# alexrenz/AdaPM

Hardware: AMD Instinct MI355X
Metric: pull_push_ops_per_s (higher is better)
Workload: dtype fp32; 1 GPU; model=kge_complex_dim512, entities=10000000, relations=1000, dim=512, neg_samples=16, global_batch=16384, triples=90000000, parallelism=ps-async-dp1, fused_step=True, warmup_extra_steps=400

## Files before the change

### adapm_amd/__init__.py

```python
from __future__ import annotations

import threading
from typing import Optional

import numpy as np
import torch

try:
    from . import _C
except ImportError as e:
    raise ImportError(
        "adapm_amd native extension not built — run `python build.py` at the repo root"
    ) from e

from . import runtime as _rt
from .sampling import SamplingManager, make_distribution
from .sync import SyncManager

TECH_ALL = 0
TECH_REPLICATION_ONLY = 1
TECH_RELOCATION_ONLY = 2

_SETUP = {}

# ... 67 lines not shown
        )
        if cfg.get("locality_stats"):
            self._s.enable_locality_stats()
        if cfg.get("trace_keys") is not None:
            tk = cfg["trace_keys"]
            t = torch.tensor([-1], dtype=torch.int64) if tk == "all" else _to_key_tensor(tk)
            self._s.enable_key_trace(t)
        self._stats_out = cfg.get("stats_out")
        self.sampling: Optional[SamplingManager] = None
        self._sync = SyncManager(self._s, rt, max_per_sec=cfg["max_sync_per_sec"],
                                 time_intent_actions=cfg["time_intent_actions"])
        self._sync.start()
        self._local_barrier = threading.Barrier(max(1, cfg["num_threads"]))
        self._num_workers = max(1, cfg["num_threads"])
        self._shut = False


    def enable_sampling_support(self, scheme: str, with_replacement: bool, distribution: str,
                                min: int, max: int, counts=None, power: float = 0.75,
                                pool_size: int = 5_000, reuse_factor: int = 4):
        d = make_distribution(distribution, min, max, seed=self.rt.rank, counts=counts,
                              power=power, device=self.rt.device)
        self.sampling = SamplingManager(self._s, scheme, with_replacement, d, min, max,
                                        pool_size=pool_size, reuse_factor=reuse_factor)

    def barrier(self):
        if self.rt.world > 1:
            with self.rt.worker_group_lock:
                torch.distributed.barrier(group=self.rt.worker_group)

    def my_rank(self) -> int:
        return self.rt.rank

    def shutdown(self):
        if self._shut:
            return
        self._shut = True
        self._sync.request_stop()
        self._sync.join()
        self._final_report()
        _rt.shutdown_runtime()

    def _final_report(self):
        import os
        import sys

        st = self.stats()
# ... 248 lines not shown
```

### adapm_amd/csrc/core.cpp

```cpp
#include <torch/extension.h>
#include <ATen/Parallel.h>

#include <algorithm>
#include <atomic>
#include <condition_variable>
#include <cstring>
#include <limits>
#include <deque>
#include <map>
#include <queue>
#include <tuple>
#include <memory>
#include <mutex>
#include <random>
#include <thread>
#include <chrono>
#include <unordered_map>
#include <unordered_set>
#include <cstdio>
#include <vector>

#include "common.h"
#include "kernels.h"
#include "ops.h"

#ifdef ADAPM_WITH_HIP
#include <c10/hip/HIPStream.h>
#endif

extern "C" {
int adapm_host_arena_alloc(long long floats, int want_device_visible, void** host_ptr,
                           void** dev_ptr);
void adapm_host_arena_free(void* host_ptr, int was_device_visible);
}

namespace adapm {

namespace py = pybind11;

static void* current_stream(const torch::Device& dev) {
#ifdef ADAPM_WITH_HIP
  if (dev.is_cuda()) return (void*)c10::hip::getCurrentHIPStream(dev.index()).stream();
#endif
  return nullptr;
}


struct Slab {
  torch::Tensor buf;
  float* data = nullptr;
// ... 142 lines not shown
  std::vector<Key> keys;
};

struct ChannelState {
  std::mutex mu;
  std::deque<IntentReq> intent_queue;
  std::vector<IntentReq> future_intents;
  struct IntentExpiry {
    Clock end;
    int wid;
    std::shared_ptr<std::vector<Key>> keys;
    bool operator>(const IntentExpiry& o) const { return end > o.end; }
  };
  std::priority_queue<IntentExpiry, std::vector<IntentExpiry>, std::greater<>> intent_expiry;
  std::unordered_set<Key> replicas;
  std::unordered_map<Key, uint64_t> holders;
  std::deque<OutRec> out_queue;
  std::vector<RespRec> responses;
  std::unordered_map<Key, uint32_t> reloc_ctr;
  std::unordered_map<Key, int64_t> reloc_round;
  std::atomic<int64_t> rounds{0};
  int64_t idle_streak = 0;
  std::atomic<int64_t> idle2_events{0};
};


class Server {
 public:
  Server(int64_t num_keys, torch::Tensor lens, int rank, int world, int num_channels,
         int num_workers, std::string device, double capacity_factor, int techniques,
         bool location_caches, int64_t device_cap_floats = 0, int64_t host_spill_floats = 0,
         double sync_threshold = 0.0)
      : num_keys_(num_keys),
        rank_(rank),
        world_(world),
        nch_(num_channels),
        techniques_(techniques),
        use_loc_cache_(location_caches),
        sync_threshold_(sync_threshold),
        dev_(device) {
    TORCH_CHECK((nch_ & (nch_ - 1)) == 0, "num_channels must be a power of 2");
    {
      int hw = (int)std::thread::hardware_concurrency();
      int nt = std::max(1, std::min(hw / std::max(1, world_) - 2, 31));
      if (const char* e = getenv("ADAPM_PASS_THREADS")) nt = std::max(1, atoi(e));
      pass_pool_.want_threads = nt;
// ... 2119 lines not shown
  bool fused_plain_ok(void* st) {
    if (clocks_.size() != 1 || fused_multi_stream_) return false;
    if (!fused_marks_.defined()) {
      if (getenv("ADAPM_FUSED_ATOMIC")) {
        fused_multi_stream_ = true;
        return false;
      }
      fused_marks_ = torch::zeros({rowmark_words(num_keys_)},
                                  torch::TensorOptions().dtype(torch::kInt32).device(dev_));
      if (getenv("ADAPM_FUSED_STATS"))
        fused_shared_stat_ =
            torch::zeros({1}, torch::TensorOptions().dtype(torch::kInt64).device(dev_));
      fused_marks_stream_ = st;
      return true;
    }
    if (st == fused_marks_stream_) return true;
#ifdef ADAPM_WITH_HIP
    hipStreamSynchronize((hipStream_t)fused_marks_stream_);
#endif
    fused_multi_stream_ = true;
    return false;
  }

  torch::Tensor kge_step_fused(torch::Tensor keys_s, torch::Tensor keys_r, torch::Tensor keys_o,
                               torch::Tensor keys_neg, int64_t N, int64_t D, double lr,
                               double eps) {
    TORCH_CHECK(world_ == 1, "kge_step_fused requires a single rank (all keys local)");
    TORCH_CHECK(uniform_len_ == 2 * D, "kge_step_fused: store rows must be [emb|accum] = 2D");
    TORCH_CHECK(layout_identity_.load(), "kge_step_fused requires the identity layout");
    TORCH_CHECK(dev_.is_cuda(), "kge_step_fused is the GPU fast path");
    for (auto* t : {&keys_s, &keys_r, &keys_o, &keys_neg}) check_keys(*t);
    int64_t B = keys_s.numel();
    TORCH_CHECK(keys_r.numel() == B && keys_o.numel() == B && keys_neg.numel() == B * N);
    auto rng_check = [&](const torch::Tensor& t) { check_key_range(t); };
    rng_check(keys_s);
    rng_check(keys_r);
    rng_check(keys_o);
    rng_check(keys_neg);

    auto loss = torch::empty({B}, torch::TensorOptions().dtype(torch::kFloat32).device(dev_));
    auto ks = keys_s.to(dev_, true);
    auto kr = keys_r.to(dev_, true);
    auto ko = keys_o.to(dev_, true);
    auto kn = keys_neg.to(dev_, true);
    void* st = current_stream(dev_);
    {
      InflightGuard g(this);
      std::unique_lock<std::mutex> mg(fused_mu_);
      if (fused_plain_ok(st)) {
        RowMarkKeys mk{{ks.data_ptr<int64_t>(), kr.data_ptr<int64_t>(), ko.data_ptr<int64_t>(),
                        kn.data_ptr<int64_t>()},
                       {B, B, B, B * N},
                       4};
        auto* marks = reinterpret_cast<uint32_t*>(fused_marks_.data_ptr<int32_t>());
        rowmark_set_gpu(marks, mk, st);
        kge_complex_step_fused_gpu(
            slab_.data, mk.keys[0], mk.keys[1], mk.keys[2], mk.keys[3], loss.data_ptr<float>(),
            (int)B, (int)N, (int)D, Slab::padded(uniform_len_), world_, rank_, (float)lr,
            (float)eps, st, marks,
            fused_shared_stat_.defined()
                ? reinterpret_cast<unsigned long long*>(fused_shared_stat_.data_ptr<int64_t>())
                : nullptr);
        rowmark_clear_gpu(marks, mk, st);
        stat_fused_plain_ += 1;
      } else {
        mg.unlock();
        kge_complex_step_fused_gpu(slab_.data, ks.data_ptr<int64_t>(), kr.data_ptr<int64_t>(),
                                   ko.data_ptr<int64_t>(), kn.data_ptr<int64_t>(),
                                   loss.data_ptr<float>(), (int)B, (int)N, (int)D,
                                   Slab::padded(uniform_len_), world_, rank_, (float)lr,
                                   (float)eps, st);
        stat_fused_atomic_ += 1;
      }
    }
    int64_t total = 3 * B + B * N;
    stat_pull_keys_ += total;
    stat_pull_local_ += total;
    stat_push_keys_ += total;
    stat_push_local_ += total;
    stat_pulls_ += 1;
    stat_pushes_ += 1;
    return loss;
  }

  struct FusedResolve {
    std::vector<std::vector<int64_t>> offs;
    std::vector<int64_t> missed;
    int64_t b_hit = 0;
  };

  FusedResolve resolve_fused(const std::vector<std::pair<const int64_t*, int>>& arrs,
                             int64_t B) {
    FusedResolve out;
    const int na = (int)arrs.size();
    constexpr int64_t G = 1024;
    int64_t nchunks = (B + G - 1) / G;
    struct Part {
      std::vector<std::vector<int64_t>> offs;
      std::vector<int64_t> missed;
    };
    std::vector<Part> parts(nchunks);
    pass_pool_.run(nchunks, [&](int64_t c0, int64_t c1) {
      for (int64_t c = c0; c < c1; ++c) {
        Part& P = parts[c];
        P.offs.resize(na);
// ... 863 lines not shown
  if (prob.is_cuda()) {
    alias_draw_gpu(prob.data_ptr<float>(), alias.data_ptr<int32_t>(), prob.numel(),
                   (uint64_t)seed, N, out.data_ptr<int64_t>(), current_stream(prob.device()));
  } else {
    alias_draw_cpu(prob.data_ptr<float>(), alias.data_ptr<int32_t>(), prob.numel(),
                   (uint64_t)seed, N, out.data_ptr<int64_t>());
  }
  return out;
}

}

PYBIND11_MODULE(TORCH_EXTENSION_NAME, m) {
  using namespace adapm;
  m.def("hip_available", &hip_available);
  m.def("kge_complex_step", &kge_complex_step, py::call_guard<py::gil_scoped_release>());
  m.def("alias_draw", &alias_draw, py::call_guard<py::gil_scoped_release>());
  m.def("rescal_step", &rescal_step, py::call_guard<py::gil_scoped_release>());
  m.def("rescal_step_grouped", &rescal_step_grouped, py::call_guard<py::gil_scoped_release>());
  m.def("kge_complex_score", &kge_complex_score, py::call_guard<py::gil_scoped_release>());
  m.def("w2v_sgns_step", &w2v_sgns_step, py::call_guard<py::gil_scoped_release>());
  m.def("mf_update_step", &mf_update_step, py::call_guard<py::gil_scoped_release>());
  m.def("mf_loss", &mf_loss, py::call_guard<py::gil_scoped_release>());
  py::class_<Server>(m, "Server")
      .def(py::init<int64_t, torch::Tensor, int, int, int, int, std::string, double, int, bool,
                    int64_t, int64_t, double>(),
           py::arg("num_keys"), py::arg("value_lengths"), py::arg("rank"), py::arg("world"),
           py::arg("num_channels"), py::arg("num_workers"), py::arg("device"),
           py::arg("capacity_factor") = 2.0, py::arg("techniques") = 0,
           py::arg("location_caches") = true, py::arg("device_cap_floats") = 0,
           py::arg("host_spill_floats") = 0, py::arg("sync_threshold") = 0.0)
      .def("pull", &Server::pull, py::call_guard<py::gil_scoped_release>())
      .def("push", &Server::push, py::call_guard<py::gil_scoped_release>())
      .def("pull_if_local", &Server::pull_if_local, py::call_guard<py::gil_scoped_release>())
      .def("is_local", &Server::is_local)
      .def("intent", &Server::intent, py::call_guard<py::gil_scoped_release>())
      .def("advance_clock", &Server::advance_clock)
      .def("current_clock", &Server::current_clock)
      .def("worker_clocks", &Server::worker_clocks)
      .def("wait", &Server::wait, py::call_guard<py::gil_scoped_release>())
      .def("wait_all", &Server::wait_all, py::call_guard<py::gil_scoped_release>())
      .def("is_finished", &Server::is_finished)
      .def("round_counts", &Server::round_counts)
      .def("wait_rounds", &Server::wait_rounds, py::call_guard<py::gil_scoped_release>())
      .def("idle_counts", &Server::idle_counts)
      .def("wait_idle", &Server::wait_idle, py::call_guard<py::gil_scoped_release>())
      .def("set_intent_ahead", &Server::set_intent_ahead)
      .def("sync_collect", &Server::sync_collect, py::call_guard<py::gil_scoped_release>())
      .def("sync_process", &Server::sync_process, py::call_guard<py::gil_scoped_release>())
      .def("sync_respond", &Server::sync_respond, py::call_guard<py::gil_scoped_release>())
      .def("sync_apply", &Server::sync_apply, py::call_guard<py::gil_scoped_release>())
      .def("sync_finish", &Server::sync_finish, py::arg("ch"),
           py::arg("globally_idle") = false, py::call_guard<py::gil_scoped_release>())
      .def("fail", &Server::fail, py::call_guard<py::gil_scoped_release>())
      .def("failed_reason", &Server::failed_reason)
      .def("scan_local", &Server::scan_local, py::call_guard<py::gil_scoped_release>())
      .def("kge_step_fused", &Server::kge_step_fused, py::call_guard<py::gil_scoped_release>())
      .def("w2v_step_fused", &Server::w2v_step_fused, py::call_guard<py::gil_scoped_release>())
      .def("mf_step_fused", &Server::mf_step_fused, py::call_guard<py::gil_scoped_release>())
      .def("kge_step_fused_general", &Server::kge_step_fused_general,
           py::call_guard<py::gil_scoped_release>())
      .def("w2v_step_fused_general", &Server::w2v_step_fused_general,
           py::call_guard<py::gil_scoped_release>())
      .def("mf_step_fused_general", &Server::mf_step_fused_general,
           py::call_guard<py::gil_scoped_release>())
      .def("rebalance_spill", &Server::rebalance_spill, py::arg("max_moves") = 4096,
           py::call_guard<py::gil_scoped_release>())
      .def("key_tier", &Server::key_tier)
      .def("get_len", &Server::get_len)
      .def("uniform_len", &Server::uniform_len)
      .def("layout_identity", &Server::layout_identity)
      .def("num_keys", &Server::num_keys)
      .def("rank", &Server::rank)
      .def("world", &Server::world)
      .def("num_channels", &Server::num_channels)
      .def("owner_hint", &Server::owner_hint)
      .def("enable_locality_stats", &Server::enable_locality_stats)
      .def("enable_key_trace", &Server::enable_key_trace)
      .def("debug_key_state", &Server::debug_key_state)
      .def("debug_set_loc_cache", &Server::debug_set_loc_cache)
// ... 7 lines not shown
```

### adapm_amd/csrc/kernels.h

```cpp
#pragma once
#include <cstdint>

namespace adapm {

void kge_complex_step_gpu(const float* s, const float* r, const float* o, const float* neg,
                          float* ds, float* dr, float* do_, float* dneg, float* loss,
                          int B, int N, int D, float lr, float eps, void* stream);
void kge_complex_step_cpu(const float* s, const float* r, const float* o, const float* neg,
                          float* ds, float* dr, float* do_, float* dneg, float* loss,
                          int B, int N, int D, float lr, float eps);

struct RowMarkKeys {
  const int64_t* keys[4];
  int64_t n[4];
  int count;
};
inline int64_t rowmark_words(int64_t rows) { return (rows + 15) / 16; }
void rowmark_set_gpu(uint32_t* marks, const RowMarkKeys& ks, void* stream);
void rowmark_clear_gpu(uint32_t* marks, const RowMarkKeys& ks, void* stream);

void kge_complex_step_fused_gpu(float* slab, const int64_t* keys_s, const int64_t* keys_r,
                                const int64_t* keys_o, const int64_t* keys_neg, float* loss,
                                int B, int N, int D, int32_t plen, int world, int rank,
                                float lr, float eps, void* stream,
// ... 33 lines not shown
void w2v_sgns_step_gpu(const float* ctr, const float* ctx, const float* neg, float* dctr,
                       float* dctx, float* dneg, float* loss, int B, int N, int D, float lr,
                       float eps, void* stream);
void w2v_sgns_step_cpu(const float* ctr, const float* ctx, const float* neg, float* dctr,
                       float* dctx, float* dneg, float* loss, int B, int N, int D, float lr,
                       float eps);

void mf_update_step_gpu(const float* w, const float* h, const float* x, float* dw, float* dh,
                        float* loss, int B, int R, float lr, float lambda, float eps,
                        void* stream);
void mf_update_step_cpu(const float* w, const float* h, const float* x, float* dw, float* dh,
                        float* loss, int B, int R, float lr, float lambda, float eps);

void mf_loss_gpu(const float* w, const float* h, const float* x, float* out2, int B, int R,
                 float lambda, void* stream);
void mf_loss_cpu(const float* w, const float* h, const float* x, float* out2, int B, int R,
                 float lambda);

void alias_draw_gpu(const float* prob, const int32_t* alias, int64_t n, uint64_t seed,
                    int64_t N, int64_t* out, void* stream);
void alias_draw_cpu(const float* prob, const int32_t* alias, int64_t n, uint64_t seed,
                    int64_t N, int64_t* out);

}

namespace adapm {


void kge_complex_score_mfma_gpu(const float* s, const float* r, const float* cand,
                                float* scores, float* qbuf, int B, int E, int D, void* stream);

void mfma_grouped_gemm_gpu(const float* S, const float* W, const float* R, float* out,
                           const int* starts, int G, int D, int sstride, int wstride,
                           int64_t rstride, int out_rstride, int64_t ostride, int mode,
                           int total_tiles, void* stream);

void rescal_mid_gpu(const float* U, const float* o, const float* neg, float* do_, float* dneg,
                    float* Wm, float* loss, int B, int N, int D, float lr, float eps,
                    void* stream);

void adagrad_rows_gpu(const float* grad, const float* rows, float* out, int64_t n_rows,
                      int dvals, int gstride, int rstride, float lr, float eps, void* stream);

}
```

### adapm_amd/csrc/kernels_cpu.cpp

```cpp
#include <cmath>
#include <vector>

#include "kernels.h"

namespace adapm {

static inline float sigmoidf_(float x) { return 1.f / (1.f + std::exp(-x)); }
static inline float softplusf_(float x) { return x > 20.f ? x : std::log1p(std::exp(x)); }

void kge_complex_step_cpu(const float* s, const float* r, const float* o, const float* neg,
                          float* ds, float* dr, float* do_, float* dneg, float* loss, int B,
                          int N, int D, float lr, float eps) {
  const int dc = D >> 1;
  const int row = D << 1;
  std::vector<float> a_sre(dc), a_sim(dc), a_rre(dc), a_rim(dc), u_re(dc), u_im(dc);
  for (int b = 0; b < B; ++b) {
    const float* sb = s + (int64_t)b * row;
    const float* rb = r + (int64_t)b * row;
    for (int k = 0; k < dc; ++k) {
      u_re[k] = sb[k] * rb[k] - sb[dc + k] * rb[dc + k];
      u_im[k] = sb[dc + k] * rb[k] + sb[k] * rb[dc + k];
      a_sre[k] = a_sim[k] = a_rre[k] = a_rim[k] = 0.f;
    }
    float lsum = 0.f;
    for (int j = 0; j <= N; ++j) {
      const float* ob = (j == 0) ? o + (int64_t)b * row : neg + ((int64_t)b * N + (j - 1)) * row;
// ... 239 lines not shown
    reg += lambda * nrm;
  }
  out2[0] += (float)se;
  out2[1] += (float)reg;
}

static inline uint64_t pcg_hash64_c(uint64_t x) {
  x ^= x >> 33; x *= 0xff51afd7ed558ccdULL;
  x ^= x >> 33; x *= 0xc4ceb9fe1a85ec53ULL;
  x ^= x >> 33;
  return x;
}

void alias_draw_cpu(const float* prob, const int32_t* alias, int64_t n, uint64_t seed,
                    int64_t N, int64_t* out) {
  for (int64_t i = 0; i < N; ++i) {
    uint64_t h = pcg_hash64_c(seed ^ (uint64_t)i * 0x9e3779b97f4a7c15ULL);
    int64_t slot = (int64_t)(h % (uint64_t)n);
    float u = (float)((h >> 40) & 0xffffff) * (1.0f / 16777216.0f);
    out[i] = (u < prob[slot]) ? slot : (int64_t)alias[slot];
  }
}

}

namespace adapm {

void rescal_step_cpu(const float* s, const float* r, const float* o, const float* neg,
                     float* ds, float* drl, float* do_, float* dneg, float* loss, int B, int N,
                     int D, float lr, float eps) {
  const int erow = 2 * D;
  const int64_t rrow = 2LL * D * D;
  std::vector<float> u(D), w(D), t(D);
  for (int b = 0; b < B; ++b) {
    const float* sb = s + (int64_t)b * erow;
    const float* rb = r + (int64_t)b * rrow;
    for (int j = 0; j < D; ++j) {
      double a = 0;
      for (int i = 0; i < D; ++i) a += rb[(int64_t)i * D + j] * sb[i];
      u[j] = (float)a;
    }
    std::fill(w.begin(), w.end(), 0.f);
    float lsum = 0.f;
    for (int j = 0; j <= N; ++j) {
      const float* ob = (j == 0) ? o + (int64_t)b * erow : neg + ((int64_t)b * N + j - 1) * erow;
      float* dob = (j == 0) ? do_ + (int64_t)b * erow : dneg + ((int64_t)b * N + j - 1) * erow;
// ... 36 lines not shown
```

### adapm_amd/csrc/kernels_hip.hip

```cpp
#include <hip/hip_runtime.h>
#include <algorithm>

#include "kernels.h"

namespace adapm {

#define KT 256

__device__ inline float block_reduce_sum(float v, float* lds) {
  for (int off = 32; off > 0; off >>= 1) v += __shfl_xor(v, off, 64);
  int wave = threadIdx.x >> 6;
  int lane = threadIdx.x & 63;
  if (lane == 0) lds[wave] = v;
  __syncthreads();
  float r = (threadIdx.x < KT / 64) ? lds[threadIdx.x] : 0.f;
  if (threadIdx.x < 64) {
    for (int off = 2; off > 0; off >>= 1) r += __shfl_xor(r, off, 64);
  }
  if (threadIdx.x == 0) lds[0] = r;
  __syncthreads();
  float out = lds[0];
  __syncthreads();
  return out;
}

__device__ inline float sigmoidf(float x) { return 1.f / (1.f + __expf(-x)); }
// ... 306 lines not shown
#undef LAUNCH
}
void mf_update_step_gpu(const float* w, const float* h, const float* x, float* dw, float* dh,
                        float* loss, int B, int R, float lr, float lambda, float eps,
                        void* stream) {
  hipLaunchKernelGGL(k_mf_step, dim3(grid_for(B)), dim3(KT), 0, (hipStream_t)stream, w, h, x, dw,
                     dh, loss, B, R, lr, lambda, eps);
}

}

namespace adapm {
void alias_draw_gpu(const float* prob, const int32_t* alias, int64_t n, uint64_t seed,
                    int64_t N, int64_t* out, void* stream) {
  if (N == 0) return;
  int blocks = (int)std::min<int64_t>((N + 255) / 256, 4096);
  hipLaunchKernelGGL(k_alias_draw, dim3(blocks), dim3(256), 0, (hipStream_t)stream, prob, alias,
                     n, seed, N, out);
}
}

namespace adapm {

__global__ void k_rescal_step(const float* __restrict__ s, const float* __restrict__ r,
                              const float* __restrict__ o, const float* __restrict__ neg,
                              float* __restrict__ ds, float* __restrict__ drl,
                              float* __restrict__ do_, float* __restrict__ dneg,
                              float* __restrict__ loss, int B, int N, int D, float lr,
                              float eps) {
  extern __shared__ __attribute__((aligned(16))) float smem[];
  float* Rm = smem;
  float* u = Rm + D * D;
  float* w = u + D;
  float* es = w + D;
  float* red = es + D;
  const int erow = 2 * D;
  const int64_t rrow = 2LL * D * D;

  for (int b = blockIdx.x; b < B; b += gridDim.x) {
    const float* sb = s + (int64_t)b * erow;
    const float* rb = r + (int64_t)b * rrow;
    for (int i = threadIdx.x; i < D * D; i += KT) Rm[i] = rb[i];
    for (int i = threadIdx.x; i < D; i += KT) {
      es[i] = sb[i];
      w[i] = 0.f;
    }
// ... 391 lines not shown
```

### adapm_amd/models/kge.py

```python
from __future__ import annotations

import dataclasses
import os
import time
from collections import defaultdict
from typing import Optional

import numpy as np
import torch

_PHASE_TIMING = os.environ.get("ADAPM_PHASE_TIMING", "0") == "1"

import adapm_amd
from adapm_amd import _C


@dataclasses.dataclass
class ComplExConfig:
    num_entities: int = 1_000_000
    num_relations: int = 1_000
    dim: int = 512
    neg_samples: int = 16
    batch_size: int = 4096
    lr: float = 0.1
    eps: float = 1e-6
    lookahead: int = 4
    init_scale: float = 0.1
    seed: int = 42

    @property
    def num_keys(self) -> int:
        return self.num_entities + self.num_relations

    @property
# ... 99 lines not shown
        pt = w.push(all_keys, all_d, async_=True)
        if pt != -1:
            self._pending.append(pt)
        if not async_push:
            w.wait(pt)
        while len(self._pending) > 64:
            w.wait(self._pending.pop(0))
        t0 = self._ph("push", t0)
        if sync_loss:
            out = float(loss.mean().item())
            self._ph("loss_sync", t0)
            return out
        return loss

    def train_batch_fused(self, triples: np.ndarray, sync_loss: bool = False,
                          force_general: bool = False):
        cfg = self.cfg
        w = self.worker
        raw = self.server.raw
        if self.dev.type != "cuda" and not force_general:
            return self.train_batch(triples, sync_loss=sync_loss)
        B = len(triples)
        s_keys, r_keys, o_keys = self.keys_of(triples)
        neg_keys = np.ascontiguousarray(self._draw_negatives(B), dtype=np.int64)

        if self.world == 1 and not force_general and raw.layout_identity():
            loss = raw.kge_step_fused(
                torch.from_numpy(s_keys), torch.from_numpy(r_keys), torch.from_numpy(o_keys),
                torch.from_numpy(neg_keys), cfg.neg_samples, cfg.dim, cfg.lr, cfg.eps)
            return float(loss.mean().item()) if sync_loss else loss

        negs2 = neg_keys.reshape(B, cfg.neg_samples)
        if self._deferred is not None:
            dtr, dng = self._deferred
            self._deferred = None
            n_def = len(dtr)
            triples = np.concatenate([dtr, triples])
            negs2 = np.concatenate([dng, negs2])
            s_keys, r_keys, o_keys = self.keys_of(triples)
            neg_keys = negs2.reshape(-1)
        else:
            n_def = 0

        loss, missed = raw.kge_step_fused_general(
            torch.from_numpy(s_keys), torch.from_numpy(r_keys), torch.from_numpy(o_keys),
            torch.from_numpy(np.ascontiguousarray(neg_keys)), cfg.neg_samples, cfg.dim,
            cfg.lr, cfg.eps)
        if missed.numel() == 0:
            return float(loss.mean().item()) if sync_loss else loss
# ... 390 lines not shown
```

### adapm_amd/sampling.py

```python
from __future__ import annotations

import threading
from dataclasses import dataclass, field
from typing import Dict, Optional

import numpy as np
import torch


class Distribution:
    def draw(self, n: int) -> np.ndarray:
        raise NotImplementedError


class Uniform(Distribution):
    def __init__(self, lo: int, hi: int, seed: int):
        self.lo, self.hi = lo, hi
        self.rng = np.random.default_rng(seed)

    def draw(self, n):
        return self.rng.integers(self.lo, self.hi, size=n, dtype=np.int64)


class LogUniform(Distribution):

    def __init__(self, lo: int, hi: int, seed: int):
        self.lo, self.hi = lo, hi
        self.rng = np.random.default_rng(seed)

    def draw(self, n):
        u = self.rng.random(n)
        k = np.exp(u * np.log(self.hi - self.lo + 1)) + self.lo - 1
        return np.minimum(k.astype(np.int64), self.hi - 1)


class Unigram(Distribution):

    def __init__(self, counts: np.ndarray, key_of: Optional[np.ndarray], power: float, seed: int,
                 device=None):
        p = counts.astype(np.float64) ** power
        p = p / p.sum()
        self.prob, self.alias = self._build_alias(p)
        self.key_of = key_of
        self.seed = np.random.default_rng(seed).integers(1, 2 ** 62)
# ... 20 lines not shown
        return (_t.from_numpy(prob.clip(0, 1).astype(np.float32)),
                _t.from_numpy(alias))

    def draw(self, n):
        from . import _C

        self._calls += 1
        out = _C.alias_draw(self.prob, self.alias, int(self.seed + self._calls), n)
        keys = out.cpu().numpy() if out.is_cuda else out.numpy()
        return keys if self.key_of is None else self.key_of[keys]


@dataclass
class _Sample:
    keys: Optional[np.ndarray]
    remaining: int
    used: set = field(default_factory=set)
    cursor: int = 0


class SamplingManager:

    def __init__(self, server, scheme: str, with_replacement: bool, dist_: Distribution,
                 lo: int, hi: int, pool_size: int = 5_000, reuse_factor: int = 4):
        self.POOL_SIZE = pool_size
        self.POOL_REUSE = reuse_factor
        self.server = server
        self.scheme = scheme
        self.with_replacement = with_replacement
        self.dist = dist_
        self.lo, self.hi = lo, hi
        self.lock = threading.Lock()
        self.samples: Dict[int, _Sample] = {}
        self.next_id = 1
        self.pool: np.ndarray = np.empty(0, dtype=np.int64)
        self.pool_uses = 0


    def prepare(self, worker, K: int, start: int, end: int) -> int:
        with self.lock:
            sid = self.next_id
            self.next_id += 1
        if self.scheme in ("naive", "preloc", "pool"):
            if self.scheme == "pool":
                keys = self._from_pool(K)
            else:
                keys = self._draw(K)
            self.samples[sid] = _Sample(keys=keys, remaining=K)
            if self.scheme == "preloc" and self.server.world() > 1:
                worker.intent(torch.from_numpy(keys), start, end)
        else:
            self.samples[sid] = _Sample(keys=None, remaining=K)
        return sid

    def pull(self, worker, sid: int, n: int):
        s = self.samples[sid]
        if s.remaining < n:
            raise ValueError(f"sample {sid}: requested {n} > remaining {s.remaining}")
        if self.scheme == "local":
            keys = self._local_draw(n, s)
        else:
            keys = s.keys[s.cursor:s.cursor + n]
            s.cursor += n
        s.remaining -= n
        return keys

    def finish(self, sid: int):
        self.samples.pop(sid, None)


    def _draw(self, n) -> np.ndarray:
        if self.with_replacement:
            return self.dist.draw(n)
        out = []
        seen = set()
        while len(out) < n:
            cand = self.dist.draw(max(2 * (n - len(out)), 16))
            for c in cand:
                c = int(c)
                if c not in seen:
                    seen.add(c)
                    out.append(c)
                    if len(out) == n:
                        break
        return np.array(out, dtype=np.int64)

    def _from_pool(self, n) -> np.ndarray:
        with self.lock:
            if len(self.pool) < n or self.pool_uses >= self.POOL_REUSE * self.POOL_SIZE:
                self.pool = self.dist.draw(max(self.POOL_SIZE, n))
                self.pool_uses = 0
# ... 43 lines not shown
```

Measured before the change: 941.9 million key-ops/s.

## Generate uniform negative samples on GPU with a bit-exact PCG64 stream

Adds a native UniformStream that reproduces numpy's PCG64 bounded-integer draw on the GPU using jump-ahead tables, a per-chunk generate kernel and a compaction kernel. The fused KGE step can then draw B*N negatives on the device instead of generating them in numpy and copying them over. Positive keys are also packed into one pinned buffer with a single range check and a single host-to-device copy, replacing four separate copies and checks. The price is substantial new RNG and state-sync code, plus stream-ownership synchronisation whenever RNG state moves between host and device.

Result: faster. 1.083 billion key-ops/s (median of 6 runs) (+15.0%).

```diff
diff --git a/adapm_amd/__init__.py b/adapm_amd/__init__.py
--- a/adapm_amd/__init__.py
+++ b/adapm_amd/__init__.py
@@ -113,7 +113,8 @@
         d = make_distribution(distribution, min, max, seed=self.rt.rank, counts=counts,
                               power=power, device=self.rt.device)
         self.sampling = SamplingManager(self._s, scheme, with_replacement, d, min, max,
-                                        pool_size=pool_size, reuse_factor=reuse_factor)
+                                        pool_size=pool_size, reuse_factor=reuse_factor,
+                                        device=self.rt.device)
 
     def barrier(self):
         if self.rt.world > 1:
diff --git a/adapm_amd/csrc/core.cpp b/adapm_amd/csrc/core.cpp
--- a/adapm_amd/csrc/core.cpp
+++ b/adapm_amd/csrc/core.cpp
@@ -23,9 +23,12 @@
 #include "common.h"
 #include "kernels.h"
 #include "ops.h"
+#include "ustream.h"
 
 #ifdef ADAPM_WITH_HIP
 #include <c10/hip/HIPStream.h>
+#include <ATen/core/CachingHostAllocator.h>
+#include <ATen/hip/impl/HIPStreamMasqueradingAsCUDA.h>
 #endif
 
 extern "C" {
@@ -214,6 +217,100 @@
   std::atomic<int64_t> rounds{0};
   int64_t idle_streak = 0;
   std::atomic<int64_t> idle2_events{0};
+};
+
+
+class UniformStream {
+ public:
+  UniformStream(int64_t lo, int64_t hi, const std::string& device)
+      : lo_(lo), hi_(hi), dev_(device) {
+    TORCH_CHECK(supported(lo, hi), "UniformStream: [", lo, ", ", hi,
+                ") is not a range of numpy's 32-bit bounded draw");
+    excl_ = (uint32_t)((uint64_t)hi - (uint64_t)lo);
+    thr_ = (uint32_t)((0x100000000ull - excl_) % excl_);
+    state_ = torch::zeros({USTREAM_STATE_WORDS},
+                          torch::TensorOptions().dtype(torch::kInt64).device(dev_));
+  }
+
+  static bool supported(int64_t lo, int64_t hi) {
+    if (hi <= lo || lo == std::numeric_limits<int64_t>::min()) return false;
+    uint64_t span = (uint64_t)hi - (uint64_t)lo;
+    return span >= 2 && span <= 0xFFFFFFFFull;
+  }
+
+  void import_state(uint64_t state_hi, uint64_t state_lo, uint64_t inc_hi, uint64_t inc_lo,
+                    uint64_t has_uint32, uint64_t uinteger) {
+    auto h = torch::empty({USTREAM_STATE_WORDS}, torch::kInt64);
+    uint64_t* p = reinterpret_cast<uint64_t*>(h.data_ptr<int64_t>());
+    p[0] = state_hi, p[1] = state_lo, p[2] = inc_hi, p[3] = inc_lo;
+    p[4] = has_uint32 ? 1 : 0, p[5] = uinteger & 0xFFFFFFFFull;
+    ustream_build_table(p);
+    std::lock_guard<std::mutex> g(mu_);
+    adopt(current_stream(dev_));
+    state_.copy_(h);
+  }
+
+  std::vector<uint64_t> export_state() {
+    torch::Tensor h;
+    {
+      std::lock_guard<std::mutex> g(mu_);
+      adopt(current_stream(dev_));
+      h = state_.slice(0, 0, USTREAM_GEN_WORDS).cpu();
+    }
+    const uint64_t* p = reinterpret_cast<const uint64_t*>(h.data_ptr<int64_t>());
+    return std::vector<uint64_t>(p, p + USTREAM_GEN_WORDS);
+  }
+
+  torch::Tensor draw(int64_t n, int64_t slack = -1) {
+    TORCH_CHECK(n >= 0, "UniformStream.draw: n must be >= 0");
+    auto opt = torch::TensorOptions().dtype(torch::kInt64).device(dev_);
+    auto out = torch::empty({n}, opt);
+    if (n == 0) return out;
+    if (slack < 0) {
+      double p = (double)thr_ / 4294967296.0;
+      double w0 = (double)n / (1.0 - p);
+      slack = (int64_t)std::ceil(w0 - (double)n + 8.0 * std::sqrt(w0 * p) / (1.0 - p)) + 16;
+    }
+    const int64_t words = n + slack;
+    std::lock_guard<std::mutex> g(mu_);
+    void* st = current_stream(dev_);
+    adopt(st);
+    auto tmp = torch::empty({ustream_tmp_words(words)}, opt);
+    uint64_t* sp = reinterpret_cast<uint64_t*>(state_.data_ptr<int64_t>());
+    if (dev_.is_cuda()) {
+#ifdef ADAPM_WITH_HIP
+      uniform_draw_gpu(sp, lo_, excl_, thr_, n, words, out.data_ptr<int64_t>(),
+                       tmp.data_ptr<int64_t>(), st);
+#else
+      TORCH_CHECK(false, "UniformStream: built without HIP");
+#endif
+    } else {
+      uniform_draw_cpu(sp, lo_, excl_, thr_, n, words, out.data_ptr<int64_t>(),
+                       tmp.data_ptr<int64_t>());
+    }
+    return out;
+  }
+
+  int64_t lo() const { return lo_; }
+  int64_t hi() const { return hi_; }
+  const torch::Device& device() const { return dev_; }
+
+ private:
+  void adopt(void* st) {
+#ifdef ADAPM_WITH_HIP
+    if (dev_.is_cuda() && have_owner_ && st != owner_) hipStreamSynchronize((hipStream_t)owner_);
+#endif
+    owner_ = st;
+    have_owner_ = true;
+  }
+
+  int64_t lo_, hi_;
+  uint32_t excl_ = 0, thr_ = 0;
+  torch::Device dev_;
+  torch::Tensor state_;
+  std::mutex mu_;
+  void* owner_ = nullptr;
+  bool have_owner_ = false;
 };
 
 
@@ -2379,36 +2476,89 @@
     return false;
   }
 
-  torch::Tensor kge_step_fused(torch::Tensor keys_s, torch::Tensor keys_r, torch::Tensor keys_o,
-                               torch::Tensor keys_neg, int64_t N, int64_t D, double lr,
-                               double eps) {
+  struct StagedKeys {
+    torch::Tensor dev;
+    std::vector<const int64_t*> ptr;
+  };
+  StagedKeys stage_keys(std::initializer_list<const torch::Tensor*> parts) {
+    int64_t total = 0;
+    for (auto* t : parts) {
+      check_keys(*t);
+      total += t->numel();
+    }
+    auto blob = torch::empty(
+        {total}, torch::TensorOptions().dtype(torch::kInt64).pinned_memory(true));
+    int64_t* dst = blob.data_ptr<int64_t>();
+    const uint64_t lim = (uint64_t)num_keys_;
+    uint64_t bad = 0;
+    for (auto* t : parts) {
+      const int64_t* kp = t->data_ptr<int64_t>();
+      const int64_t n = t->numel();
+      for (int64_t i = 0; i < n; ++i) {
+        int64_t k = kp[i];
+        dst[i] = k;
+        bad |= ((uint64_t)k >= lim);
+      }
+      dst += n;
+    }
+    if (bad)
+      for (auto* t : parts) check_key_range(*t);
+    StagedKeys sk;
+    sk.dev = torch::empty({total}, torch::TensorOptions().dtype(torch::kInt64).device(dev_));
+#ifdef ADAPM_WITH_HIP
+    auto stream = c10::hip::getCurrentHIPStreamMasqueradingAsCUDA(dev_.index());
+    TORCH_CHECK(copy_keys_gpu(sk.dev.data_ptr<int64_t>(), blob.data_ptr<int64_t>(), total,
+                              (void*)stream.stream()),
+                "kge_step_fused: the pinned key staging buffer is not visible to the device");
+    at::getHostAllocator(at::kCUDA)->record_event(
+        blob.data_ptr(), blob.storage().data_ptr().get_context(), stream.unwrap());
+#else
+    TORCH_CHECK(false, "kge_step_fused: built without HIP");
+#endif
+    const int64_t* dp = sk.dev.data_ptr<int64_t>();
+    for (auto* t : parts) {
+      sk.ptr.push_back(dp);
+      dp += t->numel();
+    }
+    return sk;
+  }
+
+  std::tuple<torch::Tensor, torch::Tensor> kge_step_fused_impl(
+      const torch::Tensor& keys_s, const torch::Tensor& keys_r, const torch::Tensor& keys_o,
+      const torch::Tensor* keys_neg, UniformStream* us, int64_t N, int64_t D, double lr,
+      double eps) {
     TORCH_CHECK(world_ == 1, "kge_step_fused requires a single rank (all keys local)");
     TORCH_CHECK(uniform_len_ == 2 * D, "kge_step_fused: store rows must be [emb|accum] = 2D");
     TORCH_CHECK(layout_identity_.load(), "kge_step_fused requires the identity layout");
     TORCH_CHECK(dev_.is_cuda(), "kge_step_fused is the GPU fast path");
-    for (auto* t : {&keys_s, &keys_r, &keys_o, &keys_neg}) check_keys(*t);
     int64_t B = keys_s.numel();
-    TORCH_CHECK(keys_r.numel() == B && keys_o.numel() == B && keys_neg.numel() == B * N);
-    auto rng_check = [&](const torch::Tensor& t) { check_key_range(t); };
-    rng_check(keys_s);
-    rng_check(keys_r);
-    rng_check(keys_o);
-    rng_check(keys_neg);
+    TORCH_CHECK(keys_r.numel() == B && keys_o.numel() == B);
+    StagedKeys sk;
+    torch::Tensor drawn;
+    const int64_t* kn;
+    if (us) {
+      TORCH_CHECK(us->lo() >= 0 && us->hi() <= num_keys_, "kge_step_fused_sampled: stream range [",
+                  us->lo(), ", ", us->hi(), ") exceeds the store's ", num_keys_, " keys");
+      TORCH_CHECK(us->device() == dev_,
+                  "kge_step_fused_sampled: stream is not on the store's device");
+      TORCH_CHECK(N >= 0 && B * N > 0, "kge_step_fused_sampled: nothing to draw");
+      sk = stage_keys({&keys_s, &keys_r, &keys_o});
+      drawn = us->draw(B * N);
+      kn = drawn.data_ptr<int64_t>();
+    } else {
+      TORCH_CHECK(keys_neg->numel() == B * N);
+      sk = stage_keys({&keys_s, &keys_r, &keys_o, keys_neg});
+      kn = sk.ptr[3];
+    }
+    const int64_t *ks = sk.ptr[0], *kr = sk.ptr[1], *ko = sk.ptr[2];
 
     auto loss = torch::empty({B}, torch::TensorOptions().dtype(torch::kFloat32).device(dev_));
-    auto ks = keys_s.to(dev_, true);
-    auto kr = keys_r.to(dev_, true);
-    auto ko = keys_o.to(dev_, true);
-    auto kn = keys_neg.to(dev_, true);
     void* st = current_stream(dev_);
     {
       InflightGuard g(this);
       std::unique_lock<std::mutex> mg(fused_mu_);
       if (fused_plain_ok(st)) {
-        RowMarkKeys mk{{ks.data_ptr<int64_t>(), kr.data_ptr<int64_t>(), ko.data_ptr<int64_t>(),
-                        kn.data_ptr<int64_t>()},
-                       {B, B, B, B * N},
-                       4};
+        RowMarkKeys mk{{ks, kr, ko, kn}, {B, B, B, B * N}, 4};
         auto* marks = reinterpret_cast<uint32_t*>(fused_marks_.data_ptr<int32_t>());
         rowmark_set_gpu(marks, mk, st);
         kge_complex_step_fused_gpu(
@@ -2422,11 +2572,9 @@
         stat_fused_plain_ += 1;
       } else {
         mg.unlock();
-        kge_complex_step_fused_gpu(slab_.data, ks.data_ptr<int64_t>(), kr.data_ptr<int64_t>(),
-                                   ko.data_ptr<int64_t>(), kn.data_ptr<int64_t>(),
-                                   loss.data_ptr<float>(), (int)B, (int)N, (int)D,
-                                   Slab::padded(uniform_len_), world_, rank_, (float)lr,
-                                   (float)eps, st);
+        kge_complex_step_fused_gpu(slab_.data, ks, kr, ko, kn, loss.data_ptr<float>(), (int)B,
+                                   (int)N, (int)D, Slab::padded(uniform_len_), world_, rank_,
+                                   (float)lr, (float)eps, st);
         stat_fused_atomic_ += 1;
       }
     }
@@ -2437,7 +2585,20 @@
     stat_push_local_ += total;
     stat_pulls_ += 1;
     stat_pushes_ += 1;
-    return loss;
+    return {loss, drawn};
+  }
+
+  torch::Tensor kge_step_fused(torch::Tensor keys_s, torch::Tensor keys_r, torch::Tensor keys_o,
+                               torch::Tensor keys_neg, int64_t N, int64_t D, double lr,
+                               double eps) {
+    return std::get<0>(
+        kge_step_fused_impl(keys_s, keys_r, keys_o, &keys_neg, nullptr, N, D, lr, eps));
+  }
+
+  std::tuple<torch::Tensor, torch::Tensor> kge_step_fused_sampled(
+      torch::Tensor keys_s, torch::Tensor keys_r, torch::Tensor keys_o, UniformStream& us,
+      int64_t N, int64_t D, double lr, double eps) {
+    return kge_step_fused_impl(keys_s, keys_r, keys_o, nullptr, &us, N, D, lr, eps);
   }
 
   struct FusedResolve {
@@ -3347,6 +3508,16 @@
   m.def("w2v_sgns_step", &w2v_sgns_step, py::call_guard<py::gil_scoped_release>());
   m.def("mf_update_step", &mf_update_step, py::call_guard<py::gil_scoped_release>());
   m.def("mf_loss", &mf_loss, py::call_guard<py::gil_scoped_release>());
+  py::class_<UniformStream>(m, "UniformStream")
+      .def(py::init<int64_t, int64_t, std::string>(), py::arg("lo"), py::arg("hi"),
+           py::arg("device"))
+      .def_static("supported", &UniformStream::supported)
+      .def("import_state", &UniformStream::import_state, py::call_guard<py::gil_scoped_release>())
+      .def("export_state", &UniformStream::export_state, py::call_guard<py::gil_scoped_release>())
+      .def("draw", &UniformStream::draw, py::arg("n"), py::arg("slack") = -1,
+           py::call_guard<py::gil_scoped_release>())
+      .def("lo", &UniformStream::lo)
+      .def("hi", &UniformStream::hi);
   py::class_<Server>(m, "Server")
       .def(py::init<int64_t, torch::Tensor, int, int, int, int, std::string, double, int, bool,
                     int64_t, int64_t, double>(),
@@ -3381,6 +3552,8 @@
       .def("failed_reason", &Server::failed_reason)
       .def("scan_local", &Server::scan_local, py::call_guard<py::gil_scoped_release>())
       .def("kge_step_fused", &Server::kge_step_fused, py::call_guard<py::gil_scoped_release>())
+      .def("kge_step_fused_sampled", &Server::kge_step_fused_sampled,
+           py::call_guard<py::gil_scoped_release>())
       .def("w2v_step_fused", &Server::w2v_step_fused, py::call_guard<py::gil_scoped_release>())
       .def("mf_step_fused", &Server::mf_step_fused, py::call_guard<py::gil_scoped_release>())
       .def("kge_step_fused_general", &Server::kge_step_fused_general,
diff --git a/adapm_amd/csrc/kernels.h b/adapm_amd/csrc/kernels.h
--- a/adapm_amd/csrc/kernels.h
+++ b/adapm_amd/csrc/kernels.h
@@ -79,6 +79,13 @@
 void alias_draw_cpu(const float* prob, const int32_t* alias, int64_t n, uint64_t seed,
                     int64_t N, int64_t* out);
 
+void uniform_draw_gpu(uint64_t* state, int64_t lo, uint32_t excl, uint32_t thr, int64_t n,
+                      int64_t words, int64_t* out, int64_t* tmp, void* stream);
+void uniform_draw_cpu(uint64_t* state, int64_t lo, uint32_t excl, uint32_t thr, int64_t n,
+                      int64_t words, int64_t* out, int64_t* tmp);
+
+bool copy_keys_gpu(int64_t* dst, const int64_t* src_host, int64_t n, void* stream);
+
 }
 
 namespace adapm {
diff --git a/adapm_amd/csrc/kernels_cpu.cpp b/adapm_amd/csrc/kernels_cpu.cpp
--- a/adapm_amd/csrc/kernels_cpu.cpp
+++ b/adapm_amd/csrc/kernels_cpu.cpp
@@ -1,7 +1,9 @@
+#include <algorithm>
 #include <cmath>
 #include <vector>
 
 #include "kernels.h"
+#include "ustream.h"
 
 namespace adapm {
 
@@ -287,6 +289,31 @@
   }
 }
 
+void uniform_draw_cpu(uint64_t* state, int64_t lo, uint32_t excl, uint32_t thr, int64_t n,
+                      int64_t words, int64_t* out, int64_t* tmp) {
+  const UStreamRange r{lo, excl, thr};
+  const int64_t chunks = ustream_chunks(words), nb = ustream_blocks(words);
+  int64_t* counts = tmp + USTREAM_TMP_COUNTS;
+  int64_t* keys = counts + nb;
+  for (int64_t b = 0; b < nb; ++b) counts[b] = 0;
+  for (int64_t c = 0; c < chunks; ++c)
+    counts[c / USTREAM_BLOCK] +=
+        ustream_gen_chunk(state, r, words, c, keys + c * USTREAM_CHUNK, 1);
+  int64_t total = 0, consumed = 0;
+  for (int64_t b = 0; b < nb; ++b) {
+    int64_t idx = total;
+    total += counts[b];
+    if (idx >= n) continue;
+    const int64_t w1 = std::min((b + 1) * (int64_t)USTREAM_BLOCK * USTREAM_CHUNK, words);
+    for (int64_t w = b * (int64_t)USTREAM_BLOCK * USTREAM_CHUNK; w < w1 && idx < n; ++w) {
+      if (keys[w] == USTREAM_REJECTED) continue;
+      out[idx++] = keys[w];
+      if (idx == n) consumed = w + 1;
+    }
+  }
+  ustream_finish(state, r, n, words, total, consumed, out);
+}
+
 }
 
 namespace adapm {
diff --git a/adapm_amd/csrc/kernels_hip.hip b/adapm_amd/csrc/kernels_hip.hip
--- a/adapm_amd/csrc/kernels_hip.hip
+++ b/adapm_amd/csrc/kernels_hip.hip
@@ -2,6 +2,7 @@
 #include <algorithm>
 
 #include "kernels.h"
+#include "ustream.h"
 
 namespace adapm {
 
@@ -354,6 +355,119 @@
 
 namespace adapm {
 
+static_assert(USTREAM_BLOCK == KT, "one chunk per thread of a KT workgroup");
+
+__device__ inline int64_t block_reduce_i64(int64_t v, int64_t* lds) {
+  for (int off = 32; off > 0; off >>= 1) v += __shfl_xor(v, off, 64);
+  if ((threadIdx.x & 63) == 0) lds[threadIdx.x >> 6] = v;
+  __syncthreads();
+  int64_t out = 0;
+  for (int i = 0; i < KT / 64; ++i) out += lds[i];
+  __syncthreads();
+  return out;
+}
+
+template <typename T>
+__device__ inline T* ustream_block_keys(T* tmp, int64_t nb, int64_t block) {
+  return tmp + USTREAM_TMP_COUNTS + nb + block * (KT * USTREAM_CHUNK) + threadIdx.x;
+}
+
+__global__ void __launch_bounds__(KT)
+k_ustream_gen(const uint64_t* __restrict__ state, UStreamRange r, int64_t words, int64_t chunks,
+              int64_t* __restrict__ tmp, int64_t nb) {
+  __shared__ int64_t lds[KT / 64];
+  const int64_t c = (int64_t)blockIdx.x * KT + threadIdx.x;
+  int64_t cnt = 0;
+  if (c < chunks)
+    cnt = ustream_gen_chunk(state, r, words, c, ustream_block_keys(tmp, nb, blockIdx.x), KT);
+  cnt = block_reduce_i64(cnt, lds);
+  if (threadIdx.x == 0) {
+    tmp[USTREAM_TMP_COUNTS + blockIdx.x] = cnt;
+  }
+}
+
+__global__ void __launch_bounds__(KT)
+k_ustream_compact(uint64_t* __restrict__ state, UStreamRange r, int64_t n, int64_t words,
+                  int64_t chunks, const int64_t* __restrict__ tmp, int64_t nb,
+                  int64_t* __restrict__ out) {
+  __shared__ int64_t lds[KT / 64];
+  __shared__ int wave_tot[KT / 64];
+  const int64_t* counts = tmp + USTREAM_TMP_COUNTS;
+  int64_t part = 0;
+  for (int64_t i = threadIdx.x; i < (int64_t)blockIdx.x; i += KT) part += counts[i];
+  const int64_t off = block_reduce_i64(part, lds);
+  const int64_t c = (int64_t)blockIdx.x * KT + threadIdx.x;
+  const bool live = off < n && c < chunks;
+  const int64_t* kc = ustream_block_keys(tmp, nb, blockIdx.x);
+  int64_t k[USTREAM_CHUNK];
+  int cnt = 0;
+#pragma unroll
+  for (int i = 0; i < USTREAM_CHUNK; ++i) {
+    k[i] = live ? kc[i * KT] : USTREAM_REJECTED;
+    cnt += (k[i] != USTREAM_REJECTED);
+  }
+  const int lane = threadIdx.x & 63, wave = threadIdx.x >> 6;
+  int incl = cnt;
+  for (int d = 1; d < 64; d <<= 1) {
+    int y = __shfl_up(incl, d, 64);
+    if (lane >= d) incl += y;
+  }
+  if (lane == 63) wave_tot[wave] = incl;
+  __syncthreads();
+  int64_t idx = off + incl - cnt;
+  for (int i = 0; i < wave; ++i) idx += wave_tot[i];
+  int64_t consumed = 0;
+#pragma unroll
+  for (int i = 0; i < USTREAM_CHUNK; ++i) {
+    if (k[i] == USTREAM_REJECTED) continue;
+    if (idx < n) {
+      out[idx] = k[i];
+      if (idx == n - 1) consumed = c * USTREAM_CHUNK + i + 1;
+    }
+    ++idx;
+  }
+  if (consumed) {
+    ustream_finish(state, r, n, words, n, consumed, out);
+  } else if (blockIdx.x == nb - 1 && threadIdx.x == 0) {
+    int64_t total = off;
+    for (int i = 0; i < KT / 64; ++i) total += wave_tot[i];
+    if (total < n) ustream_finish(state, r, n, words, total, 0, out);
+  }
+}
+
+void uniform_draw_gpu(uint64_t* state, int64_t lo, uint32_t excl, uint32_t thr, int64_t n,
+                      int64_t words, int64_t* out, int64_t* tmp, void* stream) {
+  if (n <= 0) return;
+  const UStreamRange r{lo, excl, thr};
+  const int64_t chunks = ustream_chunks(words), nb = ustream_blocks(words);
+  auto st = (hipStream_t)stream;
+  hipLaunchKernelGGL(k_ustream_gen, dim3((unsigned)nb), dim3(KT), 0, st, state, r, words, chunks,
+                     tmp, nb);
+  hipLaunchKernelGGL(k_ustream_compact, dim3((unsigned)nb), dim3(KT), 0, st, state, r, n, words,
+                     chunks, tmp, nb, out);
+}
+
+__global__ void k_copy_keys(int64_t* __restrict__ dst, const int64_t* __restrict__ src,
+                            int64_t n) {
+  int64_t i = (int64_t)blockIdx.x * KT + threadIdx.x;
+  if (i < n) dst[i] = src[i];
+}
+
+bool copy_keys_gpu(int64_t* dst, const int64_t* src_host, int64_t n, void* stream) {
+  if (n <= 0) return true;
+  void* src = nullptr;
+  if (hipHostGetDevicePointer(&src, const_cast<int64_t*>(src_host), 0) != hipSuccess || !src) {
+    (void)hipGetLastError();
+    return false;
+  }
+  hipLaunchKernelGGL(k_copy_keys, dim3((unsigned)((n + KT - 1) / KT)), dim3(KT), 0,
+                     (hipStream_t)stream, dst, static_cast<const int64_t*>(src), n);
+  return true;
+}
+}
+
+namespace adapm {
+
 __global__ void k_rescal_step(const float* __restrict__ s, const float* __restrict__ r,
                               const float* __restrict__ o, const float* __restrict__ neg,
                               float* __restrict__ ds, float* __restrict__ drl,
diff --git a/adapm_amd/csrc/ustream.h b/adapm_amd/csrc/ustream.h
--- /dev/null
+++ b/adapm_amd/csrc/ustream.h
@@ -0,0 +1,137 @@
+#pragma once
+#include <cstdint>
+
+#if defined(__HIP__)
+#define ADAPM_HD __host__ __device__
+#else
+#define ADAPM_HD
+#endif
+
+namespace adapm {
+
+typedef unsigned __int128 u128;
+
+constexpr int USTREAM_GEN_WORDS = 6;
+constexpr int USTREAM_STATE_WORDS = USTREAM_GEN_WORDS + 64 * 4;
+constexpr int USTREAM_CHUNK = 16;
+constexpr int USTREAM_BLOCK = 256;
+constexpr int64_t USTREAM_REJECTED = INT64_MIN;
+
+struct UStreamRange {
+  int64_t lo;
+  uint32_t excl;
+  uint32_t thr;
+};
+
+inline int64_t ustream_chunks(int64_t words) { return (words + USTREAM_CHUNK - 1) / USTREAM_CHUNK; }
+inline int64_t ustream_blocks(int64_t words) {
+  return (ustream_chunks(words) + USTREAM_BLOCK - 1) / USTREAM_BLOCK;
+}
+constexpr int USTREAM_TMP_COUNTS = 0;
+inline int64_t ustream_tmp_words(int64_t words) {
+  int64_t nb = ustream_blocks(words);
+  return USTREAM_TMP_COUNTS + nb + nb * USTREAM_BLOCK * USTREAM_CHUNK;
+}
+
+ADAPM_HD inline u128 ustream_mult() {
+  return ((u128)0x2360ED051FC65DA4ULL << 64) | (u128)0x4385DF649FCCF645ULL;
+}
+
+ADAPM_HD inline uint64_t ustream_output(u128 s) {
+  uint64_t hi = (uint64_t)(s >> 64), lo = (uint64_t)s;
+  uint64_t x = hi ^ lo;
+  unsigned rot = (unsigned)(hi >> 58);
+  return (x >> rot) | (x << ((64 - rot) & 63));
+}
+
+inline void ustream_build_table(uint64_t* st) {
+  u128 cur_mult = ustream_mult(), cur_plus = ((u128)st[2] << 64) | st[3];
+  uint64_t* t = st + USTREAM_GEN_WORDS;
+  for (int k = 0; k < 64; ++k, t += 4) {
+    t[0] = (uint64_t)(cur_mult >> 64), t[1] = (uint64_t)cur_mult;
+    t[2] = (uint64_t)(cur_plus >> 64), t[3] = (uint64_t)cur_plus;
+    cur_plus = (cur_mult + 1) * cur_plus;
+    cur_mult *= cur_mult;
+  }
+}
+
+ADAPM_HD inline u128 ustream_advance(const uint64_t* st, uint64_t delta) {
+  u128 s = ((u128)st[0] << 64) | st[1];
+  const uint64_t* t = st + USTREAM_GEN_WORDS;
+  for (; delta > 0; delta >>= 1, t += 4)
+    if (delta & 1) s = s * (((u128)t[0] << 64) | t[1]) + (((u128)t[2] << 64) | t[3]);
+  return s;
+}
+
+struct UStreamCursor {
+  u128 s, inc;
+  uint64_t j, out;
+  uint64_t has0, uint0;
+
+  ADAPM_HD UStreamCursor(const uint64_t* st, uint64_t j0) {
+    inc = ((u128)st[2] << 64) | st[3];
+    s = ustream_advance(st, j0);
+    j = j0;
+    out = ustream_output(s);
+    has0 = st[4];
+    uint0 = st[5];
+  }
+  ADAPM_HD uint32_t word(uint64_t v) {
+    uint64_t jj = v >> 1;
+    while (j < jj) {
+      s = s * ustream_mult() + inc;
+      out = ustream_output(s);
+      ++j;
+    }
+    if (v == 1 && has0) return (uint32_t)uint0;
+    return (v & 1) ? (uint32_t)(out >> 32) : (uint32_t)out;
+  }
+};
+
+ADAPM_HD inline uint64_t ustream_v0(const uint64_t* st) { return st[4] ? 1 : 2; }
+
+ADAPM_HD inline int64_t ustream_key(const UStreamRange& r, uint32_t u) {
+  uint64_t m = (uint64_t)u * r.excl;
+  return ((uint32_t)m >= r.thr) ? r.lo + (int64_t)(m >> 32) : USTREAM_REJECTED;
+}
+
+ADAPM_HD inline int ustream_gen_chunk(const uint64_t* st, const UStreamRange& r, int64_t words,
+                                      int64_t c, int64_t* chunk_keys, int64_t stride) {
+  const uint64_t v0 = ustream_v0(st);
+  const int64_t w0 = c * USTREAM_CHUNK;
+  UStreamCursor cur(st, (v0 + (uint64_t)w0) >> 1);
+  int cnt = 0;
+  for (int i = 0; i < USTREAM_CHUNK; ++i) {
+    int64_t w = w0 + i;
+    int64_t k = USTREAM_REJECTED;
+    if (w < words) k = ustream_key(r, cur.word(v0 + (uint64_t)w));
+    chunk_keys[i * stride] = k;
+    cnt += (k != USTREAM_REJECTED);
+  }
+  return cnt;
+}
+
+ADAPM_HD inline void ustream_finish(uint64_t* st, const UStreamRange& r, int64_t n, int64_t words,
+                                    int64_t total, int64_t consumed, int64_t* out) {
+  const uint64_t v0 = ustream_v0(st);
+  if (total < n) {
+    UStreamCursor cur(st, (v0 + (uint64_t)words) >> 1);
+    int64_t w = words;
+    while (total < n) {
+      int64_t k = ustream_key(r, cur.word(v0 + (uint64_t)w));
+      ++w;
+      if (k != USTREAM_REJECTED) out[total++] = k;
+    }
+    consumed = w;
+  }
+  const uint64_t v_end = v0 + (uint64_t)consumed;
+  const uint64_t has = v_end & 1;
+  const uint64_t steps = has ? (v_end >> 1) : (v_end >> 1) - 1;
+  u128 s = ustream_advance(st, steps);
+  st[0] = (uint64_t)(s >> 64);
+  st[1] = (uint64_t)s;
+  st[4] = has;
+  st[5] = has ? (ustream_output(s) >> 32) : 0;
+}
+
+}
diff --git a/adapm_amd/models/kge.py b/adapm_amd/models/kge.py
--- a/adapm_amd/models/kge.py
+++ b/adapm_amd/models/kge.py
@@ -10,6 +10,7 @@
 import torch
 
 _PHASE_TIMING = os.environ.get("ADAPM_PHASE_TIMING", "0") == "1"
+_HOST_NEGATIVES = os.environ.get("ADAPM_HOST_NEGATIVES", "0") == "1"
 
 import adapm_amd
 from adapm_amd import _C
@@ -155,9 +156,22 @@
             return self.train_batch(triples, sync_loss=sync_loss)
         B = len(triples)
         s_keys, r_keys, o_keys = self.keys_of(triples)
+
+        fast = self.world == 1 and not force_general and raw.layout_identity()
+        smp = self.server.sampling
+        if fast and smp is not None and not _HOST_NEGATIVES and smp.device_stream() is not None:
+            NN = B * cfg.neg_samples
+            sid = w.prepare_sample(NN, w.current_clock(), w.current_clock() + 2)
+            us = smp.pull_device(w, sid, NN, draw=False)
+            w.finish_sample(sid)
+            loss, _neg = raw.kge_step_fused_sampled(
+                torch.from_numpy(s_keys), torch.from_numpy(r_keys), torch.from_numpy(o_keys),
+                us, cfg.neg_samples, cfg.dim, cfg.lr, cfg.eps)
+            return float(loss.mean().item()) if sync_loss else loss
+
         neg_keys = np.ascontiguousarray(self._draw_negatives(B), dtype=np.int64)
 
-        if self.world == 1 and not force_general and raw.layout_identity():
+        if fast:
             loss = raw.kge_step_fused(
                 torch.from_numpy(s_keys), torch.from_numpy(r_keys), torch.from_numpy(o_keys),
                 torch.from_numpy(neg_keys), cfg.neg_samples, cfg.dim, cfg.lr, cfg.eps)
diff --git a/adapm_amd/sampling.py b/adapm_amd/sampling.py
--- a/adapm_amd/sampling.py
+++ b/adapm_amd/sampling.py
@@ -13,13 +13,71 @@
         raise NotImplementedError
 
 
+_M64 = (1 << 64) - 1
+
+
 class Uniform(Distribution):
+
     def __init__(self, lo: int, hi: int, seed: int):
         self.lo, self.hi = lo, hi
         self.rng = np.random.default_rng(seed)
+        self._native = None
+        self._native_dev = None
+        self._native_live = False
+        self._mu = threading.Lock()
 
     def draw(self, n):
-        return self.rng.integers(self.lo, self.hi, size=n, dtype=np.int64)
+        with self._mu:
+            self._to_host()
+            return self.rng.integers(self.lo, self.hi, size=n, dtype=np.int64)
+
+
+    def native_supported(self) -> bool:
+        from . import _C
+
+        if type(self.rng.bit_generator).__name__ != "PCG64":
+            return False
+        if not (-(1 << 63) <= self.lo and self.hi <= (1 << 63) - 1):
+            return False
+        return _C.UniformStream.supported(self.lo, self.hi)
+
+    def native_stream(self, device="cpu"):
+        with self._mu:
+            return self._to_native(str(device))
+
+    def draw_native(self, n: int, device="cpu", slack: int = -1):
+        if not self.native_supported():
+            return torch.from_numpy(self.draw(n))
+        with self._mu:
+            return self._to_native(str(device)).draw(n, slack)
+
+    def _to_native(self, device: str):
+        from . import _C
+
+        if self._native is not None and self._native_dev != device:
+            self._to_host()
+            self._native = None
+        if self._native is None:
+            self._native = _C.UniformStream(self.lo, self.hi, device)
+            self._native_dev = device
+        if not self._native_live:
+            st = self.rng.bit_generator.state
+            s, inc = st["state"]["state"], st["state"]["inc"]
+            self._native.import_state(s >> 64, s & _M64, inc >> 64, inc & _M64,
+                                      int(st["has_uint32"]), int(st["uinteger"]))
+            self._native_live = True
+        return self._native
+
+    def _to_host(self):
+        if not self._native_live:
+            return
+        w = self._native.export_state()
+        st = self.rng.bit_generator.state
+        st["state"] = {"state": (w[0] << 64) | w[1], "inc": (w[2] << 64) | w[3]}
+        st["has_uint32"] = int(w[4])
+        st["uinteger"] = int(w[5])
+        self.rng.bit_generator.state = st
+        self._native_live = False
 
 
 class LogUniform(Distribution):
@@ -86,7 +144,8 @@
 class SamplingManager:
 
     def __init__(self, server, scheme: str, with_replacement: bool, dist_: Distribution,
-                 lo: int, hi: int, pool_size: int = 5_000, reuse_factor: int = 4):
+                 lo: int, hi: int, pool_size: int = 5_000, reuse_factor: int = 4,
+                 device=None):
         self.POOL_SIZE = pool_size
         self.POOL_REUSE = reuse_factor
         self.server = server
@@ -94,6 +153,7 @@
         self.with_replacement = with_replacement
         self.dist = dist_
         self.lo, self.hi = lo, hi
+        self.device = None if device is None else str(device)
         self.lock = threading.Lock()
         self.samples: Dict[int, _Sample] = {}
         self.next_id = 1
@@ -131,6 +191,24 @@
 
     def finish(self, sid: int):
         self.samples.pop(sid, None)
+
+    def device_stream(self):
+        if (self.scheme != "local" or not self.with_replacement
+                or self.server.world() != 1 or not isinstance(self.dist, Uniform)
+                or self.device is None or not self.device.startswith("cuda")
+                or not self.dist.native_supported()):
+            return None
+        return self.dist.native_stream(self.device)
+
+    def pull_device(self, worker, sid: int, n: int, draw: bool = True):
+        us = self.device_stream()
+        if us is None:
+            raise RuntimeError("device pull is not available for this sampling setup")
+        s = self.samples[sid]
+        if s.remaining < n:
+            raise ValueError(f"sample {sid}: requested {n} > remaining {s.remaining}")
+        s.remaining -= n
+        return us.draw(n) if draw else us
 
 
     def _draw(self, n) -> np.ndarray:
```
